# fkluger/vanishing_points_2017

Hardware: AMD Instinct MI355X
Metric: images/sec (LSD->CNN->EM) + horizon-AUC parity, YUD-shape, 1/2/4/8 GPU (higher is better)
Workload: dtype f32 (CNN: f32 operands / accumulation / results; conv1 multiply EXACT bf16 pieces of the f32 operands (three per operand) on the bf16 matrix cores; conv2-5, fc6 and fc7 multiply scaled fp16 PAIRS of the f32 operands (22 of 24 significand bits, three exact products per f32 product) on the fp16 matrix

## Files before the change

vanishing_points_2017_amd/csrc/em_estep.hpp:

```cpp
#ifndef VPK_EM_ESTEP_HPP_
#define VPK_EM_ESTEP_HPP_

#include "em_ctx.hpp"

namespace vpk {

constexpr int RS_TT = 4;
constexpr int RS_RED_DOUBLES = RS_TT * 16 * 9;
constexpr int RS_PANEL_FLAG = 0x100;
VPK_DEV int rs_jchunk(int N) { return (N + 7) >> 3; }
VPK_DEV int rs_sstride(int jch, int W) { const int q = jch * W; return q + ((16 - q) & 31); }
VPK_DEV int rs_panel_doubles(int jch, int W) { return 8 * rs_sstride(jch, W) + 32; }
VPK_DEV int rs_row(int n, int jch, int S, int W) { const int sl = n / jch; return sl * S + (n - sl * jch) * W; }
VPK_DEV int rs_wfit(const EmCtx& c) {
    const int jch = rs_jchunk(c.N);
    for (int w = 32; w >= MT; w -= MT)
        if (rs_panel_doubles(jch, w) + 8 * RS_RED_DOUBLES <= c.wt_doubles) return w;
    return 0;
}
VPK_DEV int smooth_plan(const EmCtx& c, int M) {
    const int N = c.N;
    if (!c.prm.use_weights || M <= 0) return 0;
    const int Wp = ((M + MT - 1) / MT) * MT;
    const bool rows_ok = WAVE == 64 && nwaves() == 8 && c.smoother != 1;
    const int colw = N > WAVE ? 2 * WAVE : WAVE;
    const bool direct = (((N + colw - 1) / colw) % 8) == 0;
    if (M <= 32) {
        if (rows_ok && !direct && rs_panel_doubles(rs_jchunk(N), Wp) + 8 * RS_RED_DOUBLES <= c.wt_doubles) return 2;
        if ((long long)N * Wp <= c.wt_doubles) return 1;
    }
    if (rows_ok && !direct && (c.wt_doubles / N) / MT >= 1 && rs_wfit(c) >= MT) return 3;
    return 0;
}

struct EstepLine { double g0, g1, g2, g3, g4; };
template <int MEASURE> VPK_DEV EstepLine estep_line(const EmCtx& c, int n) {
    EstepLine g;
    g.g0 = c.drow[n]; g.g1 = c.drow[(size_t)c.ldn + n]; g.g2 = c.drow[2 * (size_t)c.ldn + n];
    if (MEASURE == VPK_DIST_ANGLE) { g.g3 = c.drow[3 * (size_t)c.ldn + n]; g.g4 = c.drow[4 * (size_t)c.ldn + n]; }
    else { g.g3 = 0.0; g.g4 = 0.0; }
    return g;
}
template <int MEASURE> VPK_DEV double estep_pair(const EstepLine& g, const Shared& sh, const double* X, int m) {
    if (MEASURE == VPK_DIST_ANGLE) {
        const double v1x = g.g0 - sh.vx[m], v1y = g.g1 - sh.vy[m];
        const double n1 = norm2(v1x, v1y);
        const double cc = 1 - fabs(dot2(v1x, v1y, g.g2, g.g3) / (n1 * g.g4));
        return cc * cc;
    } else {
        const double lv = (g.g0 * X[3 * m] + g.g1 * X[3 * m + 1]) + g.g2 * X[3 * m + 2];
        return lv * lv;
    }
}

template <int MEASURE = VPK_DIST_ANGLE>
VPK_DEVFN void estep(EmCtx& c, const double* X) {
    static_assert(MEASURE == VPK_DIST_ANGLE || MEASURE == VPK_DIST_DOTPROD, "the EM runs \"angle\" and \"dotprod\" (vp_localisation.py:196-203)");
    Shared& sh = SH();
    const int M = sh.M, N = c.N;
    const double kk = -0.5 / (sh.sigma_prior * sh.sigma_prior);
    long long tq_ = clock_ticks();
    {
        constexpr int G = VPG;
        const int gl = lane() % G;
        const int per_round = nwaves() * (WAVE / G);
        for (int m = wave_id() * (WAVE / G) + lane() / G; m < M; m += per_round) {
            double x0 = X[3 * m], x1 = X[3 * m + 1], x2 = X[3 * m + 2];
            double alpha, beta;
            vp_angles(x0, x1, alpha, beta);
            double acc = 0.0;
            for (int q = gl; q < sh.ncomp; q += G) {
                acc += mixture_term(alpha, beta, sh.pma[q], sh.pmb[q], kk) * sh.pw[q];
            }
            acc = group_sum<G>(acc);
            if (gl == 0) {
                sh.pv[m] = acc;
                if (MEASURE == VPK_DIST_ANGLE) {
                    sh.vx[m] = x0 / x2;
                    sh.vy[m] = x1 / x2;
                }
                double sm = sh.s[m];
                sm = sm > 1e-200 ? sm : 1e-200;
                sh.s[m] = sm;
                sh.k2[m] = 1.0 / sqrt(2 * PI_D * sm);
            }
        }
    }
    block_sync();
    if (tid() == 0) sh.dbuf[14] += lap(tq_);
    const int Wp = ((M + MT - 1) / MT) * MT;
    const int plan = smooth_plan(c, M);
    const bool panel = plan == 1 || plan == 2;
    const int rs_jch = rs_jchunk(N), rs_S = rs_sstride(rs_jch, Wp);
    double* wt = WT();
    constexpr int EU = 4;
    int T = 1;
    if (panel && WAVE == 64 && c.smoother != 1)
        while (T < 8 && 2 * T * N <= nthreads()) T *= 2;
    if (T > 1) {
        const int n_ = tid() / T, h = tid() - n_ * T;
        const bool on = n_ < N;
        const int n = on ? n_ : N - 1;
        const int Mh = (M + T - 1) / T;
        const int m_lo = on ? (h * Mh < M ? h * Mh : M) : 0, m_hi = on ? (m_lo + Mh < M ? m_lo + Mh : M) : 0;
        const EstepLine g = estep_line<MEASURE>(c, n);
        const double lw = c.lweight[n];
        gdp lvq = c.lvsq + n, pvq = c.pvl + n;
        double* wl = wt + (plan == 2 ? (size_t)rs_row(n, rs_jch, rs_S, Wp) : (size_t)n * Wp);
        int m = m_lo;
        for (; m + EU <= m_hi; m += EU) {
            double lv[EU], tt[EU];
#pragma unroll
            for (int u = 0; u < EU; ++u) lv[u] = estep_pair<MEASURE>(g, sh, X, m + u);
#pragma unroll
            for (int u = 0; u < EU; ++u)
                tt[u] = (exp_underflow(-(lv[u] / (2 * sh.s[m + u]))) * sh.k2[m + u]) * sh.pv[m + u];
#pragma unroll
            for (int u = 0; u < EU; ++u) {
                lvq[(size_t)(m + u) * c.ldn] = lv[u];
                wl[m + u] = tt[u];
            }
        }
        for (; m < m_hi; ++m) {
            const double lv1 = estep_pair<MEASURE>(g, sh, X, m);
            lvq[(size_t)m * c.ldn] = lv1;
            wl[m] = (exp_underflow(-(lv1 / (2 * sh.s[m]))) * sh.k2[m]) * sh.pv[m];
        }
        double pl = 0.0;
        for (int hh = 0; hh < T; ++hh) {
            const double prev = wave_bcast(pl, (lane() + WAVE - 1) & (WAVE - 1));
            if (h == hh) {
                if (hh > 0) pl = prev;
                for (m = m_lo; m < m_hi; ++m) pl += wl[m];
            }
        }
        pl = wave_bcast(pl, lane() | (T - 1));
        pl = (pl > 1e-12 || is_nan(pl)) ? pl : 1e-12;
        m = m_lo;
        for (; m + EU <= m_hi; m += EU) {
            double q[EU];
#pragma unroll
            for (int u = 0; u < EU; ++u) q[u] = wl[m + u];
#pragma unroll
            for (int u = 0; u < EU; ++u) q[u] = q[u] / pl;
#pragma unroll
            for (int u = 0; u < EU; ++u) {
                pvq[(size_t)(m + u) * c.ldn] = q[u];
                wl[m + u] = q[u] * lw;
            }
        }
        for (; m < m_hi; ++m) {
            const double q1 = wl[m] / pl;
            pvq[(size_t)m * c.ldn] = q1;
            wl[m] = q1 * lw;
        }
        if (on && h == T - 1)
            for (m = M; m < Wp; ++m) wl[m] = 0.0;
    } else
    for (int n = tid(); n < N; n += nthreads()) {
        const EstepLine g = estep_line<MEASURE>(c, n);
        gdp lvq = c.lvsq + n, pvq = c.pvl + n;
        double* wl = wt + (plan == 2 ? (size_t)rs_row(n, rs_jch, rs_S, Wp) : (size_t)n * Wp);
        double pl = 0.0;
        int m = 0;
        for (; m + EU <= M; m += EU) {
            double lv[EU], tt[EU];
#pragma unroll
            for (int u = 0; u < EU; ++u) lv[u] = estep_pair<MEASURE>(g, sh, X, m + u);
#pragma unroll
            for (int u = 0; u < EU; ++u)
                tt[u] = (exp_underflow(-(lv[u] / (2 * sh.s[m + u]))) * sh.k2[m + u]) * sh.pv[m + u];
#pragma unroll
            for (int u = 0; u < EU; ++u) {
                lvq[(size_t)(m + u) * c.ldn] = lv[u];
                if (panel) wl[m + u] = tt[u]; else pvq[(size_t)(m + u) * c.ldn] = tt[u];
                pl += tt[u];
            }
        }
        for (; m < M; ++m) {
            const double lv1 = estep_pair<MEASURE>(g, sh, X, m);
            lvq[(size_t)m * c.ldn] = lv1;
            const double t1 = (exp_underflow(-(lv1 / (2 * sh.s[m]))) * sh.k2[m]) * sh.pv[m];
            if (panel) wl[m] = t1; else pvq[(size_t)m * c.ldn] = t1;
            pl += t1;
        }
        pl = (pl > 1e-12 || is_nan(pl)) ? pl : 1e-12;
        const double lw = c.lweight[n];
        gdp ws = c.wsrc + (size_t)n * c.mcap;
        m = 0;
        for (; m + EU <= M; m += EU) {
            double q[EU];
#pragma unroll
            for (int u = 0; u < EU; ++u) q[u] = panel ? wl[m + u] : pvq[(size_t)(m + u) * c.ldn];
#pragma unroll
            for (int u = 0; u < EU; ++u) q[u] = q[u] / pl;
#pragma unroll
            for (int u = 0; u < EU; ++u) {
                pvq[(size_t)(m + u) * c.ldn] = q[u];
                if (panel) wl[m + u] = q[u] * lw;
                else ws[m + u] = q[u] * lw;
            }
        }
        for (; m < M; ++m) {
            const double q1 = (panel ? wl[m] : pvq[(size_t)m * c.ldn]) / pl;
            pvq[(size_t)m * c.ldn] = q1;
            if (panel) wl[m] = q1 * lw; else ws[m] = q1 * lw;
        }
        for (m = M; m < Wp; ++m) {
            if (panel) wl[m] = 0.0; else ws[m] = 0.0;
        }
    }
    if (plan == 2)
        for (int p = N * Wp + tid(); p < 8 * rs_jch * Wp; p += nthreads()) {
            const int j = p / Wp;
            wt[rs_row(j, rs_jch, rs_S, Wp) + (p - j * Wp)] = 0.0;
        }
    if (tid() == 0) sh.dbuf[15] += lap(tq_);
    if (tid() == 0) sh.ibuf[5] = plan == 2 ? RS_PANEL_FLAG + Wp : (plan == 1 ? Wp : 0);
    block_sync();
}

}
#endif
```

Before: 22510.

## Skip exp evaluation for underflowing line-VP pairs in E-step via bitmasks

The panel E-step now first computes the squared residuals and builds a per-line bitmask of vanishing points whose exponent would not underflow. Only the kept pairs get the exp, k2 and pv products, the partial sum and the division. Underflowed pairs get an exact-zero posterior, and non-finite or sign-mismatched k2/pv entries are forced into the kept set. The goal is to cut exp and divide work when most pairs underflow, at the cost of mask bookkeeping, data-dependent loops and more divergence.

```diff
diff --git a/vanishing_points_2017_amd/csrc/em_estep.hpp b/vanishing_points_2017_amd/csrc/em_estep.hpp
--- a/vanishing_points_2017_amd/csrc/em_estep.hpp
+++ b/vanishing_points_2017_amd/csrc/em_estep.hpp
@@ -50,6 +50,99 @@
     } else {
         const double lv = (g.g0 * X[3 * m] + g.g1 * X[3 * m + 1]) + g.g2 * X[3 * m + 2];
         return lv * lv;
+    }
+}
+
+constexpr double ESTEP_UNDERFLOW_BOUND = 746.0 * (1.0 + 0x1p-40);
+typedef unsigned long long vpmask_t;
+VPK_DEV int lowest_vp(vpmask_t r) { return __builtin_ctzll(r); }
+VPK_DEV bool estep_zero_safe(double k2, double pv) {
+    return fabs(k2) <= 1.7976931348623157e308 && fabs(pv) <= 1.7976931348623157e308 &&
+           (__double_as_longlong(k2) < 0) == (__double_as_longlong(pv) < 0);
+}
+VPK_DEV vpmask_t estep_zero_safe_mask(const Shared& sh, int M) {
+    if (WAVE == MAXM) {
+        const int m = lane() < M ? lane() : 0;
+        return wave_ballot(lane() < M && estep_zero_safe(sh.k2[m], sh.pv[m]));
+    }
+    vpmask_t r = 0;
+    for (int m = 0; m < M; ++m) r |= (vpmask_t)estep_zero_safe(sh.k2[m], sh.pv[m]) << m;
+    return r;
+}
+VPK_DEV double exp_underflow_select(double x) {
+    const double e = exp(x);
+    return x < -746.0 ? 0.0 : e;
+}
+template <int MEASURE>
+VPK_DEV vpmask_t estep_keep(const EstepLine& g, const Shared& sh, const double* X, int m_lo, int m_hi, vpmask_t force,
+                            gdp lvq, int ldn, double* wl) {
+    constexpr int EU = 4;
+    const int cnt = m_hi - m_lo;
+    const vpmask_t range = cnt <= 0 ? 0ull : ((cnt >= 64 ? ~0ull : (1ull << cnt) - 1ull) << m_lo);
+    vpmask_t keep = force & range;
+    int m = m_lo;
+    for (; m + EU <= m_hi; m += EU) {
+        double lv[EU], bound[EU];
+#pragma unroll
+        for (int u = 0; u < EU; ++u) lv[u] = estep_pair<MEASURE>(g, sh, X, m + u);
+#pragma unroll
+        for (int u = 0; u < EU; ++u) bound[u] = (2 * sh.s[m + u]) * ESTEP_UNDERFLOW_BOUND;
+#pragma unroll
+        for (int u = 0; u < EU; ++u) {
+            lvq[(size_t)(m + u) * ldn] = lv[u];
+            wl[m + u] = lv[u];
+            keep |= (vpmask_t)(!(lv[u] > bound[u])) << (m + u);
+        }
+    }
+    for (; m < m_hi; ++m) {
+        const double lv1 = estep_pair<MEASURE>(g, sh, X, m);
+        lvq[(size_t)m * ldn] = lv1;
+        wl[m] = lv1;
+        keep |= (vpmask_t)(!(lv1 > (2 * sh.s[m]) * ESTEP_UNDERFLOW_BOUND)) << m;
+    }
+    return keep;
+}
+template <bool SUM> VPK_DEV double estep_terms(vpmask_t keep, const Shared& sh, double* wl, double pl) {
+    vpmask_t r = keep;
+    while (r != 0) {
+        const int m0 = lowest_vp(r);
+        r &= r - 1;
+        const bool two = r != 0;
+        const int m1 = two ? lowest_vp(r) : m0;
+        r &= r - 1;
+        const double a0 = -(wl[m0] / (2 * sh.s[m0])), a1 = -(wl[m1] / (2 * sh.s[m1]));
+        const double t0 = (exp_underflow_select(a0) * sh.k2[m0]) * sh.pv[m0];
+        const double t1 = (exp_underflow_select(a1) * sh.k2[m1]) * sh.pv[m1];
+        wl[m0] = t0;
+        if (SUM) pl += t0;
+        if (two) {
+            wl[m1] = t1;
+            if (SUM) pl += t1;
+        }
+    }
+    return pl;
+}
+VPK_DEV void estep_posteriors(vpmask_t keep, int m_lo, int m_hi, double pl, double lw, gdp pvq, int ldn, double* wl) {
+    const double z = 0.0 / pl, zl = z * lw;
+    for (int m = m_lo; m < m_hi; ++m)
+        if (!((keep >> m) & 1)) {
+            pvq[(size_t)m * ldn] = z;
+            wl[m] = zl;
+        }
+    vpmask_t r = keep;
+    while (r != 0) {
+        const int m0 = lowest_vp(r);
+        r &= r - 1;
+        const bool two = r != 0;
+        const int m1 = two ? lowest_vp(r) : m0;
+        r &= r - 1;
+        const double q0 = wl[m0] / pl, q1 = wl[m1] / pl;
+        pvq[(size_t)m0 * ldn] = q0;
+        wl[m0] = q0 * lw;
+        if (two) {
+            pvq[(size_t)m1 * ldn] = q1;
+            wl[m1] = q1 * lw;
+        }
     }
 }
 
@@ -94,8 +187,10 @@
     const int rs_jch = rs_jchunk(N), rs_S = rs_sstride(rs_jch, Wp);
     double* wt = WT();
     constexpr int EU = 4;
+    const bool sparse = panel && c.smoother != 1;
+    const vpmask_t force = ~estep_zero_safe_mask(sh, M);
     int T = 1;
-    if (panel && WAVE == 64 && c.smoother != 1)
+    if (sparse && WAVE == 64)
         while (T < 8 && 2 * T * N <= nthreads()) T *= 2;
     if (T > 1) {
         const int n_ = tid() / T, h = tid() - n_ * T;
@@ -107,55 +202,31 @@
         const double lw = c.lweight[n];
         gdp lvq = c.lvsq + n, pvq = c.pvl + n;
         double* wl = wt + (plan == 2 ? (size_t)rs_row(n, rs_jch, rs_S, Wp) : (size_t)n * Wp);
-        int m = m_lo;
-        for (; m + EU <= m_hi; m += EU) {
-            double lv[EU], tt[EU];
-#pragma unroll
-            for (int u = 0; u < EU; ++u) lv[u] = estep_pair<MEASURE>(g, sh, X, m + u);
-#pragma unroll
-            for (int u = 0; u < EU; ++u)
-                tt[u] = (exp_underflow(-(lv[u] / (2 * sh.s[m + u]))) * sh.k2[m + u]) * sh.pv[m + u];
-#pragma unroll
-            for (int u = 0; u < EU; ++u) {
-                lvq[(size_t)(m + u) * c.ldn] = lv[u];
-                wl[m + u] = tt[u];
-            }
-        }
-        for (; m < m_hi; ++m) {
-            const double lv1 = estep_pair<MEASURE>(g, sh, X, m);
-            lvq[(size_t)m * c.ldn] = lv1;
-            wl[m] = (exp_underflow(-(lv1 / (2 * sh.s[m]))) * sh.k2[m]) * sh.pv[m];
-        }
+        const vpmask_t keep = estep_keep<MEASURE>(g, sh, X, m_lo, m_hi, force, lvq, c.ldn, wl);
+        estep_terms<false>(keep, sh, wl, 0.0);
         double pl = 0.0;
         for (int hh = 0; hh < T; ++hh) {
             const double prev = wave_bcast(pl, (lane() + WAVE - 1) & (WAVE - 1));
             if (h == hh) {
                 if (hh > 0) pl = prev;
-                for (m = m_lo; m < m_hi; ++m) pl += wl[m];
+                for (vpmask_t r = keep; r != 0; r &= r - 1) pl += wl[lowest_vp(r)];
             }
         }
         pl = wave_bcast(pl, lane() | (T - 1));
         pl = (pl > 1e-12 || is_nan(pl)) ? pl : 1e-12;
-        m = m_lo;
-        for (; m + EU <= m_hi; m += EU) {
-            double q[EU];
-#pragma unroll
-            for (int u = 0; u < EU; ++u) q[u] = wl[m + u];
-#pragma unroll
-            for (int u = 0; u < EU; ++u) q[u] = q[u] / pl;
-#pragma unroll
-            for (int u = 0; u < EU; ++u) {
-                pvq[(size_t)(m + u) * c.ldn] = q[u];
-                wl[m + u] = q[u] * lw;
-            }
-        }
-        for (; m < m_hi; ++m) {
-            const double q1 = wl[m] / pl;
-            pvq[(size_t)m * c.ldn] = q1;
-            wl[m] = q1 * lw;
-        }
+        estep_posteriors(keep, m_lo, m_hi, pl, lw, pvq, c.ldn, wl);
         if (on && h == T - 1)
-            for (m = M; m < Wp; ++m) wl[m] = 0.0;
+            for (int m = M; m < Wp; ++m) wl[m] = 0.0;
+    } else if (sparse)
+    for (int n = tid(); n < N; n += nthreads()) {
+        const EstepLine g = estep_line<MEASURE>(c, n);
+        gdp lvq = c.lvsq + n, pvq = c.pvl + n;
+        double* wl = wt + (plan == 2 ? (size_t)rs_row(n, rs_jch, rs_S, Wp) : (size_t)n * Wp);
+        const vpmask_t keep = estep_keep<MEASURE>(g, sh, X, 0, M, force, lvq, c.ldn, wl);
+        double pl = estep_terms<true>(keep, sh, wl, 0.0);
+        pl = (pl > 1e-12 || is_nan(pl)) ? pl : 1e-12;
+        estep_posteriors(keep, 0, M, pl, c.lweight[n], pvq, c.ldn, wl);
+        for (int m = M; m < Wp; ++m) wl[m] = 0.0;
     } else
     for (int n = tid(); n < N; n += nthreads()) {
         const EstepLine g = estep_line<MEASURE>(c, n);
```

New measurement: 22770 (median of 6 runs). 1.01x the previous value.
